# automerge/automerge-classic

Measured on NVIDIA H100. Metric: ops/sec applied (1M-op text trace), higher is better.
Workload: dtype int64

## Files before the change

### automerge_classic_b200/csrc/engine.cuh

```cuda
#pragma once
#include <algorithm>
#include <array>
#include <functional>
#include <initializer_list>
#include <map>
#include <memory>
#include <thread>
#include <zlib.h>
#include "patch.cuh"
#include "inflate.cuh"
#include "encode.cuh"
#include "prims.cuh"
#include "domlocal.cuh"
#include "doccols.cuh"
#include "history.cuh"
#include "unknowncols.hpp"

namespace amg {

struct DocBufs {
  DBuf<u64> id, obj, key; DBuf<u32> keyStrOff, keyStrLen, flags, valLen, valOff, time;
  void ensure(Ctx& c, size_t n, size_t keep = 0) {
    id.ensure(c, n, keep); obj.ensure(c, n, keep); key.ensure(c, n, keep); keyStrOff.ensure(c, n, keep); keyStrLen.ensure(c, n, keep);
    flags.ensure(c, n, keep); valLen.ensure(c, n, keep); valOff.ensure(c, n, keep); time.ensure(c, n, keep);
// ... 13 lines not shown
  size_t propsOff = 0, numProps = 0, editsOff = 0, numEdits = 0, elemOff = 0, valBytesOff = 0, valBytesLen = 0, bigEnd = 0;
  const u8* bytes = nullptr; size_t bytesLen = 0;
};

struct HostChange { u32 off, len; };

struct HostArena {
  HBuf<u8> buf; size_t len = 0;
  u8* data() { return buf.p; } const u8* data() const { return buf.p; }
  size_t size() const { return len; }
  void reserve(size_t n) { buf.ensure(n + 64); }
  void resize(size_t n) { if (n > len) buf.ensure(n + 64); len = n; }
  void append(const void* p, size_t n) { const size_t at = len; resize(len + n); memcpy(buf.p + at, p, n); }
  void assign(const HostArena& o) { resize(o.len); if (o.len) memcpy(buf.p, o.buf.p, o.len); }
};

inline std::string hex_of(const u8* p, size_t n) { static const char* d = "0123456789abcdef"; std::string s; for (size_t i = 0; i < n; i++) { s.push_back(d[p[i] >> 4]); s.push_back(d[p[i] & 15]); } return s; }

class Engine {
 public:
  Ctx ctx;
  DBuf<u8> arena; size_t arenaLen = 0; HostArena hostArena;
  DBuf<u8> hashes; size_t numApplied = 0;
  DocBufs doc; size_t numRows = 0; DBuf<u32> succOff; DBuf<u64> succ; size_t numSucc = 0;
  DBuf<ActorSlot> actorSlots; size_t actorCap = 0;
  DBuf<u32> actorRank;
  std::vector<std::string> actorIds;
  std::vector<u64> clock;
  std::vector<std::array<u8, 32>> heads; std::vector<u32> headIdx;
  std::vector<std::pair<u32, u32>> actorRep;
  std::vector<HostChange> changes;
  std::vector<std::array<u8, 32>> changeHashes;
  struct OrigRange { u32 idx; HostChange range; };
  std::vector<OrigRange> deflatedOriginal;
  const HostChange* originalOf(u32 idx) const {
    auto it = std::lower_bound(deflatedOriginal.begin(), deflatedOriginal.end(), idx, [](const OrigRange& a, u32 v) { return a.idx < v; });
    return it != deflatedOriginal.end() && it->idx == idx ? &it->range : nullptr;
  }
  std::vector<HostChange> queue, queueOriginal;
  u64 maxOp = 0;
  float lastPhaseMs[24] = {0};
  struct PhaseTimer* curTimer = nullptr; std::function<void()> curHostMark;
  std::vector<std::pair<const char*, float>> dbgMarks; std::function<void(const char*)> dbgMark = [](const char*) {};
  HBuf<u8> patchBuf;
  DBuf<u32> chOff, chLen, nOps, nPreds, nDeps, nActors, colOff, colLen, depBase, depIdx, primary, pass, flagWord, appRank, opBase, predBase, timeBase, amapBase, amap, authorSlot, newSlots;
  DBuf<u8> applied; DBuf<ChangeHot> hot; DBuf<ChangeMeta> meta ; DBuf<u64> errWord; DBuf<u32> hashTable;
  DBuf<u32> inflCap, inflCapOff, inflOvf; DBuf<u8> inflScratch;
  DBuf<u32> rawBase, rawPredBase, decErr, decDirect; DBuf<u64> decCursor; size_t lastDeflCount = 0, lastDeflStart = 0;
  u32* decTotalsPtr() { return reinterpret_cast<u32*>(decCursor.p + 2); }
  DBuf<u32> patchByteLen, patchByteOff; DBuf<u8> patchBytesD;
  DBuf<u32> r_objActor, r_objCtr, r_keyActor, r_keyCtr, r_keyStrOff, r_keyStrLen, r_insert, r_action, r_valLen, r_valOff, r_predNum, r_predOff, r_predActor, r_predCtr;
  DBuf<u64> o_id, o_obj, o_key, o_predId; DBuf<u32> o_keyStrOff, o_keyStrLen, o_flags, o_valLen, o_valOff, o_predOff, o_predNum, o_change, o_time;
  DBuf<u32> isRow, rowSlot, rowOfOp; DocBufs work, sorted;
  DBuf<u64> idKeys; DBuf<u32> idVals; DBuf<u32> objRow, elemRow, parentRow, keySlot, repList, repCount, listPos, perm, pos;
  DBuf<KeySlot> keySlots; DBuf<u64> sortKeys; DBuf<u32> sortVals; SortTemp sortTmp; ScanTemp scanTmp;
  ParColumnDecoder parCols{ctx, scanTmp}; size_t parDocMinRows = 4096;
  DBuf<u32> eNext, eRank, insItems, itemIdx, objSlot; DBuf<u64> ePacked, ePacked2;
  DBuf<u64> pairKey, pairSucc, newSucc; DBuf<u32> pairIdx, pairPos, pairTime, succCnt, newSuccCnt, newSuccOff, firstNewSucc;
  DBuf<u32> elemPos, keyRankAt, objPos, head, headScan, groupOf, groupRows, groupVisible, groupFirst, groupTouched, groupLinked, objTouchedAt, linkDone, emit, marker, slot;
  DBuf<u32> isObjHead, objIdx, objStart, elemVis, elemVisScan, rowEmit, firstVis, state, nItems, itemBase, qIndex, zero, wzero, zscan, wscan, editObjKey;
  DBuf<DomItem> items, items2; DBuf<PropRec> propOut; DBuf<EditRec> editOut, editOut2; DBuf<u64> editElem, editElem2;
  std::unique_ptr<ColumnEncoder> encoder; DBuf<long long> saveVals; DBuf<u32> saveStrOff, saveStrLen; std::string loadedDoc; size_t numLoaded = 0; HostChange loadedCols[9] = {}; DBuf<u64> counterTotal; DBuf<int> domW, domW2; DBuf<u32> elemMinT, editRowPos, editRowPos2, editObjKey2, rowClass, firstBare, counterOwner, newSuccTime, counterLast, runHeadFlag, runScan, runStart, elemFollower, domTw, domTw2, oldVisScan, inflLen, inflOff, groupHasChild, gCount, gElem, gT1, gQOrd, gBase, nQ, elemHasRecs, listLinkTime, editElemPos, editElemPos2, editKind, editPred, editDead, editMerge, editMulti, editLive;
  DBuf<u32> seqSlot, actorCnt, actorBaseD, clockD, changeActor, editTime; DBuf<u8> hashTmp; DBuf<u32> headsPack, headsOut; bool batchInOrder = true;
  DBuf<u32> finalTime, gFailed, memberFinal, opAt, runHead, opGroupHead; DBuf<u64> gBound; DocRows workView{}; DBuf<HostChange> chPairs; DBuf<u32> largeFlag, largeSlot, largeList; size_t lastNumLarge = 0; DBuf<u64> zwScan; DBuf<u32> deflList, patchTriples;

  explicit Engine(int device) {
    ctx.device = device;
#ifndef AMG_EMU
    int count = 0; cudaError_t e = cudaGetDeviceCount(&count);
    if (e != cudaSuccess || count == 0) throw Error(AMG_ERR_CUDA, "amgpu: no CUDA device available (this library has no CPU fallback)");
    CUDA_CHECK(cudaSetDevice(device));
    cudaDeviceProp prop; CUDA_CHECK(cudaGetDeviceProperties(&prop, device)); ctx.numSMs = prop.multiProcessorCount;
    CUDA_CHECK(cudaStreamCreateWithFlags(&ctx.stream, cudaStreamNonBlocking));
    CUDA_CHECK(cudaStreamCreateWithFlags(&ctx.side, cudaStreamNonBlocking));
    CUDA_CHECK(cudaStreamCreateWithFlags(&ctx.copy, cudaStreamNonBlocking));
    ctx.peekCap = 1u << 20; CUDA_CHECK(cudaMallocHost((void**)&ctx.peekBuf, ctx.peekCap + 64));
    ctx.peekFlag = reinterpret_cast<volatile unsigned long long*>(ctx.peekBuf + ctx.peekCap); *ctx.peekFlag = 0;
    CUDA_CHECK(cudaEventCreateWithFlags(&ctx.evUp, cudaEventDisableTiming)); CUDA_CHECK(cudaEventCreateWithFlags(&ctx.evMirror, cudaEventDisableTiming));
    CUDA_CHECK(cudaEventCreateWithFlags(&ctx.evFork, cudaEventDisableTiming)); CUDA_CHECK(cudaEventCreateWithFlags(&ctx.evJoin, cudaEventDisableTiming));
    ShaConsts k; memcpy(k.k, SHA_K, sizeof(SHA_K)); CUDA_CHECK(cudaMemcpyToSymbol(c_sha, &k, sizeof(k)));
#endif
    errWord.ensure(ctx, 4); flagWord.ensure(ctx, 16);
    actorCap = 64; actorSlots.ensure(ctx, actorCap); resetActorSlots(0, actorCap);
    succOff.ensure(ctx, 1); dev_memset(ctx, succOff.p, 0, 4);
  }
  ~Engine() {
#ifndef AMG_EMU
    if (ctx.stream) cudaStreamDestroy(ctx.stream);
    mirror_wait(ctx);
    if (ctx.side) cudaStreamDestroy(ctx.side);
    if (ctx.copy) cudaStreamDestroy(ctx.copy);
    if (ctx.peekBuf) cudaFreeHost(ctx.peekBuf);
    if (ctx.phaseEvReady) for (auto& e : ctx.phaseEv) cudaEventDestroy(e);
    if (last_peek_ctx() == &ctx) last_peek_ctx() = nullptr;
    if (ctx.evUp) cudaEventDestroy(ctx.evUp);
    if (ctx.evMirror) cudaEventDestroy(ctx.evMirror);
    if (ctx.evFork) cudaEventDestroy(ctx.evFork);
    if (ctx.evJoin) cudaEventDestroy(ctx.evJoin);
#endif
  }

  void rebuildActorTable() {
    std::vector<ActorSlot> t(actorCap); for (auto& s : t) { s.hash = 0; s.first = ~0ULL; s.actorNum = EMPTY32; s.repOff = 0; s.repLen = 0; s.pad = 0; }
    for (size_t a = 0; a < actorIds.size(); a++) {
      const u64 h = fnv1a64((const u8*)actorIds[a].data(), (u32)actorIds[a].size()); u64 s = mix64(h) & (actorCap - 1);
      while (t[s].hash != 0) s = (s + 1) & (actorCap - 1);
      t[s].hash = h; t[s].first = 0; t[s].actorNum = (u32)a; t[s].repOff = actorRep[a].first; t[s].repLen = actorRep[a].second;
    }
    h2d(ctx, actorSlots.p, t.data(), actorCap * sizeof(ActorSlot)); sync(ctx);
  }
// ... 138 lines not shown
```

### automerge_classic_b200/csrc/engine_impl.cuh

```cuda
#pragma once
#include <chrono>
#ifndef AMG_EMU
#include <nvtx3/nvToolsExt.h>
#endif
#include "engine.cuh"
#include "misc.cuh"

namespace amg {

#ifdef AMG_EMU
#define CUDA_CHECK_EMU(x) do {} while (0)
#else
#define CUDA_CHECK_EMU(x) CUDA_CHECK(x)
#endif
static const size_t PATCH_HDR_WORDS = 20;
struct NvtxPhases {
#ifndef AMG_EMU
  bool open = false;
  void next(const char* name) { if (open) nvtxRangePop(); open = name != nullptr; if (name) nvtxRangePushA(name); }
  ~NvtxPhases() { if (open) nvtxRangePop(); }
#else
  void next(const char*) {}
#endif
};
// ... 466 lines not shown
    if (!inOrder) {
      perm.ensure(ctx, B + 1); dev_memset(ctx, perm.p, 0, (B + 1) * 4);
      foreach(ctx, B, OpsInOrderKernel{nOps.p, applied.p, appRank.p, perm.p});
      scan_exclusive(ctx, scanTmp, perm.p, perm.p, numNew);
    }
    foreach(ctx, B, TimeBaseKernel{perm.p, applied.p, appRank.p, opBaseP, inOrder ? 1 : 0, timeBase.p});
    DBuf<u64>& maxOpD = pairSucc; maxOpD.ensure(ctx, 1); h2d(ctx, maxOpD.p, &maxOpNow, 8);
    foreach(ctx, B, MaxOpKernel{hot.p, nOps.p, applied.p, decErr.p, maxOpD.p, errWord.p});
    d2h(ctx, &maxOpNow, maxOpD.p, 8);
    RawRows raw = rawRows();
    lastNumLarge = 0;
    if (anyLarge) {
      largeFlag.ensure(ctx, B + 1); largeSlot.ensure(ctx, B + 2); largeList.ensure(ctx, B + 1);
      foreach(ctx, B, LargeFlagKernel{nOps.p, applied.p, largeFlag.p});
      scan_exclusive(ctx, scanTmp, largeFlag.p, largeSlot.p, B);
      lastNumLarge = readU32(largeSlot.p + B);
      if (lastNumLarge > 0) {
        foreach(ctx, B, CompactKernel{largeFlag.p, largeSlot.p, largeList.p});
        u32 hugeMask = 0;
        if (lastNumLarge <= 8) hugeMask = decodeHugeChanges(raw, lastNumLarge);
        foreach(ctx, (size_t)NCOLS * lastNumLarge, DecodeColumnKernel{arena.p, largeList.p, lastNumLarge, hot.p, nOps.p, nPreds.p, rawBase.p, rawPredBase.p, applied.p, raw, errWord.p, hugeDone.p});
        (void)hugeMask;
      }
    }
    for (DBuf<u64>* b : {&o_id, &o_obj, &o_key}) b->ensure(ctx, M + 1);
    o_predId.ensure(ctx, P + 1);
    for (DBuf<u32>* b : {&o_keyStrOff, &o_keyStrLen, &o_flags, &o_valLen, &o_valOff, &o_predOff, &o_predNum, &o_change, &o_time}) b->ensure(ctx, M + 1);
    OpRows ops{o_id.p, o_obj.p, o_key.p, o_keyStrOff.p, o_keyStrLen.p, o_flags.p, o_valLen.p, o_valOff.p, o_predOff.p, o_predNum.p, o_change.p, o_time.p, o_predId.p};
    foreach(ctx, M, FinalizeOpsKernel{B, hot.p, nActors.p, opBaseP, predBaseP, rawBase.p, rawPredBase.p, timeBase.p, amapBase.p, amap.p, applied.p, raw, ops, errWord.p});
    checkErr(actorsNow);
    dbgMark("decode:finalized");
    timer.mark(); hostMark(); nvtx.next("opset");
    if (maxOpNow >= (1ULL << 40)) throw Error(AMG_ERR_UNSUPPORTED, "amgpu: op counters above 2^40");
    const int ordBits = bits_for(maxOpNow) + rb;
    isRow.ensure(ctx, M + 1); rowSlot.ensure(ctx, M + 1); rowOfOp.ensure(ctx, M + 1);
    foreach(ctx, M, RowFlagKernel{o_flags.p, isRow.p}); scan_exclusive(ctx, scanTmp, isRow.p, rowSlot.p, M);
    const size_t R = readU32(rowSlot.p + M); N = numRows + R;
    if (N >= (1u << 29)) throw Error(AMG_ERR_UNSUPPORTED, "amgpu: more than 2^29 document rows");
    doc.ensure(ctx, N + 1, numRows);
    DocRows w = doc.view();
    foreach(ctx, M, AppendRowsKernel{ops, isRow.p, rowSlot.p, numRows, w, rowOfOp.p});
    const size_t icap = pow2_at_least(2 * N + 2); idKeys.ensure(ctx, icap); idVals.ensure(ctx, icap); dev_memset(ctx, idKeys.p, 0, icap * 8);
    idt = IdTable{idKeys.p, idVals.p, (u64)icap - 1};
    foreach(ctx, N, IdInsertKernel{w.id, idt, errWord.p});
    objRow.ensure(ctx, N + 1); elemRow.ensure(ctx, N + 1); parentRow.ensure(ctx, N + 1);
    foreach(ctx, N, ResolveRowsKernel{w, idt, ord, numRows, objRow.p, elemRow.p, parentRow.p, errWord.p});
    checkErr(actorsNow);
    dbgMark("opset:resolved");
    const size_t kcap = pow2_at_least(2 * N + 2); keySlots.ensure(ctx, kcap); keySlot.ensure(ctx, N + 1); repList.ensure(ctx, N + 1); repCount.ensure(ctx, 4);
    foreach(ctx, kcap, KeySlotInitKernel{keySlots.p});
    foreach(ctx, N, KeyInternKernel{arena.p, w, keySlots.p, (u64)kcap - 1, keySlot.p});
    dev_memset(ctx, repCount.p, 0, 16);
    foreach(ctx, N, KeyVerifyKernel{arena.p, w, keySlots.p, keySlot.p, repList.p, repCount.p, errWord.p});
    u32 rc[2]; readU32x2(repCount.p, repCount.p + 1, &rc[0], &rc[1]);
    const size_t D = rc[0]; const u32 maxKeyLen = rc[1];
    dbgMark("opset:keys-interned");
    if (D > 0) {
      sortKeys.ensure(ctx, D); sortVals.ensure(ctx, D);
      d2d(ctx, sortVals.p, repList.p, D * 4);
      const int chunks = (int)((maxKeyLen + 6) / 7);
      for (int ch = std::max(chunks, 1) - 1; ch >= 0; ch--) {
        foreach(ctx, D, KeyChunkKernel{arena.p, w, sortVals.p, (u32)ch * 7, sortKeys.p});
        sortPairs(sortKeys, sortVals, D, 64);
      }
      foreach(ctx, D, KeyRankKernel{sortVals.p, keySlot.p, keySlots.p});
    }
    listPos.ensure(ctx, N + 1); insItems.ensure(ctx, N + 1); emit.ensure(ctx, N + 1); slot.ensure(ctx, N + 2);
    foreach(ctx, N, InsertFlagKernel{w, emit.p}); scan_exclusive(ctx, scanTmp, emit.p, slot.p, N);
    const size_t I = readU32(slot.p + N);
    dbgMark("opset:inserts-counted");
    if (I > 0) {
      const int parentBits = bits_for(N) + 1;
      if (ordBits + parentBits > 64) throw Error(AMG_ERR_UNSUPPORTED, "amgpu: opId range x document size exceeds the 64-bit sibling sort key");
      foreach(ctx, N, CompactKernel{emit.p, slot.p, insItems.p});
      sortKeys.ensure(ctx, I); sortVals.ensure(ctx, I);
      foreach(ctx, I, SiblingKeyKernel{w, insItems.p, parentRow.p, objRow.p, ord, ordBits, sortKeys.p, errWord.p});
      d2d(ctx, sortVals.p, insItems.p, I * 4);
      sortPairs(sortKeys, sortVals, I, ordBits + parentBits);
      checkErr(actorsNow);
      itemIdx.ensure(ctx, N + 1); objSlot.ensure(ctx, N + 2);
      foreach(ctx, I, ItemIndexKernel{sortVals.p, itemIdx.p});
      foreach(ctx, N, ListObjFlagKernel{w, emit.p}); scan_exclusive(ctx, scanTmp, emit.p, objSlot.p, N);
      const size_t Lo = readU32(objSlot.p + N);
      const size_t S = 2 * I + 2 * Lo; eNext.ensure(ctx, S + 1); eRank.ensure(ctx, S + 1); ePacked.ensure(ctx, S + 1); ePacked2.ensure(ctx, S + 1);
      foreach(ctx, S, EulerInitKernel{eNext.p, eRank.p});
      foreach(ctx, I, EulerLinkKernel{sortKeys.p, ordBits, itemIdx.p, objSlot.p, eNext.p, eRank.p, I});
      foreach(ctx, S, ListRankPackKernel{eNext.p, eRank.p, ePacked.p});
      const int rounds = bits_for(S);
      for (int k = 0; k < rounds; k++) {
        foreach(ctx, S, ListRankPackedKernel{ePacked.p, ePacked2.p});
        std::swap(ePacked.p, ePacked2.p); std::swap(ePacked.cap, ePacked2.cap);
      }
      foreach(ctx, S, ListRankUnpackKernel{ePacked.p, eRank.p});
      foreach(ctx, N, ListPosKernel{eRank.p, elemRow.p, objRow.p, itemIdx.p, objSlot.p, (u32)I, listPos.p});
    } else dev_memset(ctx, listPos.p, 0, (N + 1) * 4);
    checkErr(actorsNow);
    dbgMark("opset:list-ranked");
    perm.ensure(ctx, N + 1); pos.ensure(ctx, N + 1); sortKeys.ensure(ctx, N);
    foreach(ctx, N, IotaKernel{perm.p});
    const int fieldBits[3] = {ordBits + 1, bits_for(N), ordBits + 1};
    for (int f = 0; f < 3; f++) {
      foreach(ctx, N, DocKeyKernel{f, w, perm.p, listPos.p, keySlots.p, keySlot.p, ord, sortKeys.p});
      sortPairs(sortKeys, perm, N, fieldBits[f]);
    }
    foreach(ctx, N, InversePermKernel{perm.p, pos.p});
    dbgMark("opset:doc-ordered(enqueued)");
    numPairs = numSucc + P;
    pairKey.ensure(ctx, numPairs + 1); pairSucc.ensure(ctx, numPairs + 1); pairIdx.ensure(ctx, numPairs + 1); pairPos.ensure(ctx, numPairs + 1); pairTime.ensure(ctx, numPairs + 1);
    foreach(ctx, M, DelElemCheckKernel{ops, idt, w, errWord.p});
    checkErr(actorsNow);
    foreach(ctx, numRows, OldPairsKernel{succOff.p, succ.p, pos.p, ord, pairKey.p, pairIdx.p, pairSucc.p, pairPos.p, pairTime.p});
    foreach(ctx, M, PredPairsKernel{ops, idt, pos.p, rowOfOp.p, w, elemRow.p, keySlot.p, ord, pairKey.p, pairIdx.p, pairSucc.p, pairPos.p, pairTime.p, numSucc, errWord.p});
    foreach(ctx, M, DelKeyCheckKernel{arena.p, ops, idt, w, errWord.p});
    foreach(ctx, M, IncCheckKernel{ops, idt, w, arena.p, errWord.p});
    {
      const u64 w2 = fetchErr();
      if (w2) {
        if ((w2 & 0xff) == KE_PRED_MISSING) { u64 pid = 0; d2h(ctx, &pid, o_predId.p + (w2 >> 8), 8); sync(ctx); actorIds.swap(actorsNow); std::string t = opIdText(pid); actorIds.swap(actorsNow); throw Error(AMG_ERR_RANGE, "no matching operation for pred: " + t); }
        if ((w2 & 0xff) == KE_UNKNOWN_COUNTER) { u64 oid = 0; d2h(ctx, &oid, o_id.p + (w2 >> 8), 8); sync(ctx); actorIds.swap(actorsNow); std::string t = opIdText(oid); actorIds.swap(actorsNow); throw Error(AMG_ERR_RANGE, "increment operation " + t + " for unknown counter"); }
        throwKernelError(w2, actorsNow);
      }
    }
    sortPairs(pairKey, pairIdx, numPairs, ordBits);
    foreach(ctx, numPairs, PairPosKeyKernel{pairPos.p, pairIdx.p, pairKey.p});
    sortPairs(pairKey, pairIdx, numPairs, bits_for(N));
    succCnt.ensure(ctx, N + 2); newSuccCnt.ensure(ctx, N + 2); newSuccOff.ensure(ctx, N + 2); firstNewSucc.ensure(ctx, N + 2); newSucc.ensure(ctx, numPairs + 1);
    dev_memset(ctx, succCnt.p, 0, (N + 2) * 4); dev_memset(ctx, newSuccCnt.p, 0, (N + 2) * 4); dev_memset(ctx, firstNewSucc.p, 0xff, (N + 2) * 4);
    foreach(ctx, numPairs, CountSuccKernel{pairPos.p, succCnt.p});
    foreach(ctx, numPairs, NewSuccFlagKernel{pairPos.p, pairTime.p, newSuccCnt.p});
    foreach(ctx, numPairs, FirstSuccTimeKernel{pairPos.p, pairTime.p, firstNewSucc.p});
    scan_exclusive(ctx, scanTmp, succCnt.p, newSuccOff.p, N);
    newSuccTime.ensure(ctx, numPairs + 1);
    foreach(ctx, numPairs, WriteSuccKernel{pairIdx.p, pairSucc.p, newSucc.p, pairTime.p, newSuccTime.p});
    sorted.ensure(ctx, N + 1);
    foreach(ctx, N, GatherRowsKernel{w, sorted.view(), perm.p});
    dbgMark("opset:succ+gather(enqueued)");
    timer.mark(); hostMark(); nvtx.next("patch");
    if (wantPatch) {
      objPos.ensure(ctx, N + 1);
      foreach(ctx, N, ObjPosKernel{perm.p, objRow.p, pos.p, objPos.p});
      workView = w;
      buildPatch(sorted.view(), N, false, &ops, M, &idt, rowOfOp.p, pos.p, actorsNow, out, newSuccOff.p, newSucc.p);
    }
    checkErr(actorsNow);
    timer.mark(); hostMark(); nvtx.next("heads+commit");
    dbgMark("commit:begin");
    {
      DBuf<u32>& isDep = groupLinked; isDep.ensure(ctx, G + 1); dev_memset(ctx, isDep.p, 0, (G + 1) * 4);
      foreach(ctx, B, MarkDepsKernel{applied.p, nDeps.p, depBase.p, depIdx.p, isDep.p});
      emit.ensure(ctx, B + 1); slot.ensure(ctx, B + 2); objStart.ensure(ctx, B + 1);
      foreach(ctx, B, HeadFlag2Kernel{applied.p, isDep.p, numApplied, emit.p});
      scan_exclusive(ctx, scanTmp, emit.p, slot.p, B);
      foreach(ctx, B, CompactKernel{emit.p, slot.p, objStart.p});
      const u32 nOld = (u32)headIdx.size(); u32 cap = 64, nh = 0; std::vector<u32> pack;
      headsPack.ensure(ctx, nOld + 1);
      if (nOld) h2d(ctx, headsPack.p, headIdx.data(), nOld * 4);
      for (;;) {
        const size_t words = 1 + (size_t)nOld + 9 * (size_t)cap;
// ... 1071 lines not shown
```

### automerge_classic_b200/csrc/opset.cuh

```cuda
#pragma once
#include "gate.cuh"

namespace amg {

static const u32 ROW_NONE = 0xffffffffu;
static const u32 ACT_MAKE_MAP = 0, ACT_SET = 1, ACT_MAKE_LIST = 2, ACT_DEL = 3, ACT_MAKE_TEXT = 4, ACT_INC = 5, ACT_MAKE_TABLE = 6, ACT_LINK = 7;

struct DocRows {
  u64 *id, *obj, *key; u32 *keyStrOff, *keyStrLen, *flags, *valLen, *valOff, *time;
};

struct Ord {
  const u32* actorRank; int rb;
  HD u64 operator()(u64 id) const { return (id_ctr(id) << rb) | (u64)actorRank[id_actor(id)]; }
};

struct RowFlagKernel {
  const u32* flags; u32* isRow;
  HD void operator()(size_t i) const { isRow[i] = flags_action(flags[i]) != ACT_DEL ? 1u : 0u; }
};
struct AppendRowsKernel {
  OpRows ops; const u32* isRow; const u32* rowSlot ; size_t numOld; DocRows w; u32* rowOfOp;
  HD void operator()(size_t i) const {
    if (!isRow[i]) { rowOfOp[i] = ROW_NONE; return; }
// ... 46 lines not shown
      } else {
        er = id_lookup(t, key);
        if (er == ROW_NONE || w.obj[er] != obj || !(w.flags[er] & F_INSERT)) { if (r >= numOld) raise(errWord, KE_REF_ELEM, r); er = ROW_NONE; }
      }
    }
    elemRow[r] = er; parentRow[r] = pr;
  }
};

struct KeySlot { u64 hash; u32 rep; u32 rank; };
struct KeyInternKernel {
  const u8* arena; DocRows w; KeySlot* slots; u64 mask; u32* keySlot;
  HD void operator()(size_t r) const {
    if (w.keyStrLen[r] == NULL32) { keySlot[r] = ROW_NONE; return; }
    u64 h = fnv1a64(arena + w.keyStrOff[r], w.keyStrLen[r]) ^ ((u64)w.keyStrLen[r] << 48); if (h == 0) h = 1;
    u64 s = mix64(h) & mask;
    while (true) {
      const u64 cur = atomic_cas(&slots[s].hash, (u64)0, h);
      if (cur == 0 || cur == h) { atomic_min(&slots[s].rep, (u32)r); keySlot[r] = (u32)s; return; }
      s = (s + 1) & mask;
    }
  }
};
struct KeyVerifyKernel {
  const u8* arena; DocRows w; const KeySlot* slots; const u32* keySlot; u32* repList; u32* repCount ; u64* errWord;
  HD void operator()(size_t r) const {
    const u32 s = keySlot[r]; if (s == ROW_NONE) return;
    const u32 rep = slots[s].rep;
    if (rep == (u32)r) { repList[atomic_add(repCount, 1u)] = (u32)r; atomic_max(repCount + 1, w.keyStrLen[r]); return; }
    const u32 len = w.keyStrLen[r];
    bool same = len == w.keyStrLen[rep];
    for (u32 i = 0; same && i < len; i++) same = arena[w.keyStrOff[r] + i] == arena[w.keyStrOff[rep] + i];
    if (!same) raise(errWord, KE_HASH_COLLISION, r);
  }
};
HD u64 key_chunk(const u8* s, u32 len, u32 pos) {
  u64 v = 0; u32 n = 0;
  for (u32 i = 0; i < 7; i++) {
    u32 b = 0;
    if (pos + i < len) { b = s[pos + i]; n++; if (b == 0xEE || b == 0xEF) b += 5; else if (b >= 0xF0 && b <= 0xF4) b -= 2; }
    v = (v << 8) | b;
  }
  return (v << 8) | n;
}
struct KeyChunkKernel {
  const u8* arena; DocRows w; const u32* items ; u32 pos; u64* chunk;
  HD void operator()(size_t j) const { const u32 r = items[j]; chunk[j] = key_chunk(arena + w.keyStrOff[r], w.keyStrLen[r], pos); }
};
struct KeyRankKernel {
  const u32* items; const u32* keySlot; KeySlot* slots;
  HD void operator()(size_t j) const { slots[keySlot[items[j]]].rank = (u32)j; }
};

struct IotaKernel { u32* out; HD void operator()(size_t i) const { out[i] = (u32)i; } };
struct FillU32Kernel { u32* out; u32 v; HD void operator()(size_t i) const { out[i] = v; } };
struct FillU64Kernel { u64* out; u64 v; HD void operator()(size_t i) const { out[i] = v; } };
struct GatherU64Kernel { const u64* src; const u32* idx; u64* out; HD void operator()(size_t i) const { out[i] = src[idx[i]]; } };
struct InversePermKernel { const u32* perm; u32* inv; HD void operator()(size_t i) const { inv[perm[i]] = (u32)i; } };
struct HeadFlagKernel { const u64* a; const u64* b; u32* flag; HD void operator()(size_t j) const { flag[j] = (j == 0 || a[j] != a[j - 1] || (b && b[j] != b[j - 1])) ? 1u : 0u; } };

struct SiblingKeyKernel {
  DocRows w; const u32* items; const u32* parentRow; const u32* objRow; Ord ord; int ordBits; u64* key; u64* errWord;
  HD void operator()(size_t j) const {
    const u32 r = items[j]; const u32 pr = parentRow[r];
    if (pr == ROW_NONE && objRow[r] == ROW_NONE) { raise(errWord, KE_UNSUPPORTED_OP, r); key[j] = 0; return; }
    if (pr == ROW_NONE) { const u32 a = flags_action(w.flags[objRow[r]]); if (a != ACT_MAKE_LIST && a != ACT_MAKE_TEXT) { raise(errWord, KE_UNSUPPORTED_OP, r); key[j] = 0; return; } }
    const u64 parentCode = pr != ROW_NONE ? ((u64)pr << 1) : (((u64)objRow[r] << 1) | 1);
    const u64 maxOrd = (1ULL << ordBits) - 1;
    key[j] = (parentCode << ordBits) | (maxOrd - ord(w.id[r]));
  }
};
struct ListObjFlagKernel { DocRows w; u32* flag; HD void operator()(size_t r) const { const u32 a = flags_action(w.flags[r]); flag[r] = (a == ACT_MAKE_LIST || a == ACT_MAKE_TEXT) ? 1u : 0u; } };
struct ItemIndexKernel { const u32* items; u32* itemIdx; HD void operator()(size_t j) const { itemIdx[items[j]] = (u32)j; } };
struct EulerLinkKernel {
  const u64* key; int ordBits; const u32* itemIdx; const u32* objSlot; u32* next ; u32* weight; size_t n;
  HD void operator()(size_t j) const {
    const u64 pc = key[j] >> ordBits;
    const bool firstOfParent = j == 0 || (key[j - 1] >> ordBits) != pc, lastOfParent = j + 1 == n || (key[j + 1] >> ordBits) != pc;
    const u32 parentEnter = (pc & 1) ? (u32)(2 * n + 2 * objSlot[pc >> 1]) : 2 * itemIdx[pc >> 1], parentExit = parentEnter + 1;
    if (firstOfParent) next[parentEnter] = (u32)(2 * j);
    next[2 * j + 1] = lastOfParent ? parentExit : (u32)(2 * j + 2);
    weight[2 * j] = 1;
  }
};
struct EulerInitKernel {
  u32* next; u32* weight;
  HD void operator()(size_t s) const { next[s] = (s & 1) ? (u32)s : (u32)s + 1; weight[s] = 0; }
};
struct ListRankPackKernel { const u32* next; const u32* rank; u64* packed; HD void operator()(size_t s) const { packed[s] = (u64)next[s] | ((u64)rank[s] << 32); } };
struct ListRankPackedKernel {
  const u64* in; u64* out;
  HD void operator()(size_t s) const {
    const u64 me = in[s]; const u32 n = (u32)me;
    if (n == (u32)s) { out[s] = me; return; }
    const u64 nb = in[n];
    out[s] = (u64)(u32)nb | ((u64)((u32)(me >> 32) + (u32)(nb >> 32)) << 32);
  }
};
struct ListRankUnpackKernel { const u64* packed; u32* rank; HD void operator()(size_t s) const { rank[s] = (u32)(packed[s] >> 32); } };
struct ListPosKernel {
  const u32* rank; const u32* elemRow; const u32* objRow; const u32* itemIdx; const u32* objSlot; u32 numItems; u32* listPos;
  HD void operator()(size_t r) const {
    const u32 e = elemRow[r];
    if (e == ROW_NONE || objRow[e] == ROW_NONE) { listPos[r] = 0; return; }
    listPos[r] = rank[2 * (size_t)numItems + 2 * objSlot[objRow[e]]] - rank[2 * (size_t)itemIdx[e]];
  }
};

struct DocKeyKernel {
  int field; DocRows w; const u32* perm; const u32* listPos; const KeySlot* keySlots; const u32* keySlot; Ord ord; u64* key;
  HD void operator()(size_t j) const {
    const u32 r = perm[j]; u64 k;
    if (field == 0) k = (w.keyStrLen[r] == NULL32 && (w.flags[r] & F_INSERT)) ? 0 : ord(w.id[r]) + 1;
    else if (field == 1) k = w.keyStrLen[r] == NULL32 ? listPos[r] : keySlots[keySlot[r]].rank;
    else k = w.obj[r] == 0 ? 0 : ord(w.obj[r]) + 1;
    key[j] = k;
  }
};
struct GatherRowsKernel {
  DocRows src, dst; const u32* perm;
  HD void operator()(size_t p) const {
    const u32 r = perm[p];
    dst.id[p] = src.id[r]; dst.obj[p] = src.obj[r]; dst.key[p] = src.key[r]; dst.keyStrOff[p] = src.keyStrOff[r]; dst.keyStrLen[p] = src.keyStrLen[r];
    dst.flags[p] = src.flags[r]; dst.valLen[p] = src.valLen[r]; dst.valOff[p] = src.valOff[r]; dst.time[p] = src.time[r];
  }
};

struct PredPairsKernel {
  OpRows ops; IdTable t; const u32* pos ; const u32* rowOfOp; DocRows w; const u32* elemRow; const u32* keySlot;
  Ord ord; u64* pairKey ; u32* pairIdx; u64* pairSucc; u32* pairPos; u32* pairTime; size_t pairBase; u64* errWord;
  HD void operator()(size_t i) const {
    const u32 n = ops.predNum[i];
    for (u32 j = 0; j < n; j++) {
      const size_t p = ops.predOff[i] + j; const size_t q = pairBase + p;
      const u32 target = id_lookup(t, ops.predId[p]);
      pairKey[q] = ord(ops.id[i]); pairIdx[q] = (u32)q; pairSucc[q] = ops.id[i]; pairTime[q] = ops.time[i];
      if (target == ROW_NONE || (ops.flags[i] & F_INSERT)) { raise(errWord, KE_PRED_MISSING, p); pairPos[q] = 0; continue; }
      bool ok = w.obj[target] == ops.obj[i] && w.time[target] < ops.time[i] && ord(ops.predId[p]) < ord(ops.id[i]);
      if (ops.keyStrLen[i] != NULL32) {
        ok = ok && w.keyStrLen[target] != NULL32;
        const u32 r = rowOfOp[i];
        if (ok && r != ROW_NONE) ok = keySlot[r] == keySlot[target];
      } else {
        ok = ok && w.keyStrLen[target] == NULL32 && elemRow[target] != ROW_NONE && w.id[elemRow[target]] == ops.key[i];
      }
      if (!ok) raise(errWord, KE_PRED_MISSING, p);
      pairPos[q] = pos[target];
    }
  }
};
struct IncCheckKernel {
  OpRows ops; IdTable t; DocRows w; const u8* arena; u64* errWord;
  HD void operator()(size_t i) const {
    const u32 act = flags_action(ops.flags[i]), tag = ops.valLen[i] & 15;
    if ((act == ACT_INC || (act == ACT_SET && tag == 8)) && (tag == 3 || tag == 4 || tag == 8 || tag == 9)) {
      ByteReader r(arena, ops.valOff[i], ops.valOff[i] + (ops.valLen[i] >> 4));
      if (tag == 3) r.uleb(); else r.sleb();
      if (r.err) raise(errWord, r.err, i);
    }
    if (act != ACT_INC) return;
    if (tag > 4 && tag != 8 && tag != 9) { raise(errWord, KE_UNSUPPORTED_OP, i); return; }
    bool ok = false, other = false;
    for (u32 j = 0; j < ops.predNum[i]; j++) {
      const u32 target = id_lookup(t, ops.predId[ops.predOff[i] + j]);
      if (target != ROW_NONE && flags_action(w.flags[target]) == ACT_SET && (w.valLen[target] & 15) == 8) ok = true; else other = true;
    }
    if (!ok) raise(errWord, KE_UNKNOWN_COUNTER, i);
    else if (other) raise(errWord, KE_UNSUPPORTED_OP, i);
  }
// ... 42 lines not shown
```

Baseline: 151.7 million.

## Replace pointer-jumping list ranking and three-pass doc sort with splitter tour walk and placement

Result: faster. 162.0 million (median of 6 runs) (+6.8%).

```diff
diff --git a/automerge_classic_b200/csrc/engine.cuh b/automerge_classic_b200/csrc/engine.cuh
--- a/automerge_classic_b200/csrc/engine.cuh
+++ b/automerge_classic_b200/csrc/engine.cuh
@@ -89,10 +89,11 @@
   DBuf<u32> r_objActor, r_objCtr, r_keyActor, r_keyCtr, r_keyStrOff, r_keyStrLen, r_insert, r_action, r_valLen, r_valOff, r_predNum, r_predOff, r_predActor, r_predCtr;
   DBuf<u64> o_id, o_obj, o_key, o_predId; DBuf<u32> o_keyStrOff, o_keyStrLen, o_flags, o_valLen, o_valOff, o_predOff, o_predNum, o_change, o_time;
   DBuf<u32> isRow, rowSlot, rowOfOp; DocBufs work, sorted;
-  DBuf<u64> idKeys; DBuf<u32> idVals; DBuf<u32> objRow, elemRow, parentRow, keySlot, repList, repCount, listPos, perm, pos;
+  DBuf<u64> idKeys; DBuf<u32> idVals; DBuf<u32> objRow, elemRow, parentRow, keySlot, repList, repCount, perm, pos;
   DBuf<KeySlot> keySlots; DBuf<u64> sortKeys; DBuf<u32> sortVals; SortTemp sortTmp; ScanTemp scanTmp;
   ParColumnDecoder parCols{ctx, scanTmp}; size_t parDocMinRows = 4096;
-  DBuf<u32> eNext, eRank, insItems, itemIdx, objSlot; DBuf<u64> ePacked, ePacked2;
+  DBuf<u32> insItems, restItems, itemIdx, objSlot, childCnt, sibFlag, sibSlot, tourNext, tourW, tourRank; DBuf<u64> tourOwn;
+  DBuf<u32> objFlag, objFlagScan, objHead, objHeadScan, objRankOf, objElems, objRestStart, objCount, objBase;
   DBuf<u64> pairKey, pairSucc, newSucc; DBuf<u32> pairIdx, pairPos, pairTime, succCnt, newSuccCnt, newSuccOff, firstNewSucc;
   DBuf<u32> elemPos, keyRankAt, objPos, head, headScan, groupOf, groupRows, groupVisible, groupFirst, groupTouched, groupLinked, objTouchedAt, linkDone, emit, marker, slot;
   DBuf<u32> isObjHead, objIdx, objStart, elemVis, elemVisScan, rowEmit, firstVis, state, nItems, itemBase, qIndex, zero, wzero, zscan, wscan, editObjKey;
diff --git a/automerge_classic_b200/csrc/engine_impl.cuh b/automerge_classic_b200/csrc/engine_impl.cuh
--- a/automerge_classic_b200/csrc/engine_impl.cuh
+++ b/automerge_classic_b200/csrc/engine_impl.cuh
@@ -542,9 +542,21 @@
     foreach(ctx, N, KeyInternKernel{arena.p, w, keySlots.p, (u64)kcap - 1, keySlot.p});
     dev_memset(ctx, repCount.p, 0, 16);
     foreach(ctx, N, KeyVerifyKernel{arena.p, w, keySlots.p, keySlot.p, repList.p, repCount.p, errWord.p});
-    u32 rc[2]; readU32x2(repCount.p, repCount.p + 1, &rc[0], &rc[1]);
-    const size_t D = rc[0]; const u32 maxKeyLen = rc[1];
-    dbgMark("opset:keys-interned");
+    emit.ensure(ctx, N + 1); slot.ensure(ctx, N + 2); insItems.ensure(ctx, N + 1); restItems.ensure(ctx, N + 1); objSlot.ensure(ctx, N + 2);
+    foreach(ctx, N, InsertFlagKernel{w, emit.p}); scan_exclusive(ctx, scanTmp, emit.p, slot.p, N);
+    foreach(ctx, N, SplitRowsKernel{emit.p, slot.p, insItems.p, restItems.p});
+    const SiblingParent par{w, parentRow.p, objRow.p};
+    childCnt.ensure(ctx, 2 * N + 1); sibFlag.ensure(ctx, N + 1); sibSlot.ensure(ctx, N + 2);
+    dev_memset(ctx, childCnt.p, 0, 2 * N * 4);
+    foreach(ctx, N, SiblingCountKernel{par, emit.p, childCnt.p, errWord.p});
+    foreach(ctx, N, SiblingFlagKernel{par, emit.p, childCnt.p, sibFlag.p}); scan_exclusive(ctx, scanTmp, sibFlag.p, sibSlot.p, N);
+    foreach(ctx, N, ListObjFlagKernel{w, emit.p}); scan_exclusive(ctx, scanTmp, emit.p, objSlot.p, N);
+    objFlag.ensure(ctx, 2 * N + 1); objFlagScan.ensure(ctx, 2 * N + 2); objRankOf.ensure(ctx, 2 * N + 1);
+    dev_memset(ctx, objFlag.p, 0, 2 * N * 4);
+    foreach(ctx, N, ObjEntryFlagKernel{w, objRow.p, objFlag.p}); scan_exclusive(ctx, scanTmp, objFlag.p, objFlagScan.p, 2 * N);
+    u32 cnt[6]; { void* dst[6] = {&cnt[0], &cnt[1], &cnt[2], &cnt[3], &cnt[4], &cnt[5]}; readWords({{repCount.p, 4}, {repCount.p + 1, 4}, {slot.p + N, 4}, {objSlot.p + N, 4}, {objFlagScan.p + 2 * N, 4}, {sibSlot.p + N, 4}}, dst); }
+    const size_t D = cnt[0]; const u32 maxKeyLen = cnt[1]; const size_t I = cnt[2], Lo = cnt[3], numObjEntries = cnt[4], numSib = cnt[5], numRest = N - I;
+    dbgMark("opset:counted");
     if (D > 0) {
       sortKeys.ensure(ctx, D); sortVals.ensure(ctx, D);
       d2d(ctx, sortVals.p, repList.p, D * 4);
@@ -555,45 +567,73 @@
       }
       foreach(ctx, D, KeyRankKernel{sortVals.p, keySlot.p, keySlots.p});
     }
-    listPos.ensure(ctx, N + 1); insItems.ensure(ctx, N + 1); emit.ensure(ctx, N + 1); slot.ensure(ctx, N + 2);
-    foreach(ctx, N, InsertFlagKernel{w, emit.p}); scan_exclusive(ctx, scanTmp, emit.p, slot.p, N);
-    const size_t I = readU32(slot.p + N);
-    dbgMark("opset:inserts-counted");
+    if (numObjEntries > 0) {
+      sortKeys.ensure(ctx, numObjEntries); sortVals.ensure(ctx, numObjEntries); objHead.ensure(ctx, numObjEntries + 1); objHeadScan.ensure(ctx, numObjEntries + 1);
+      foreach(ctx, 2 * N, CompactKernel{objFlag.p, objFlagScan.p, sortVals.p});
+      foreach(ctx, numObjEntries, ObjEntryKeyKernel{w, sortVals.p, ord, sortKeys.p});
+      sortPairs(sortKeys, sortVals, numObjEntries, ordBits);
+      foreach(ctx, numObjEntries, HeadFlagKernel{sortKeys.p, nullptr, objHead.p}); scan_exclusive(ctx, scanTmp, objHead.p, objHeadScan.p, numObjEntries);
+      foreach(ctx, numObjEntries, ObjRankKernel{sortVals.p, objHead.p, objHeadScan.p, objRankOf.p});
+    }
     if (I > 0) {
       const int parentBits = bits_for(N) + 1;
       if (ordBits + parentBits > 64) throw Error(AMG_ERR_UNSUPPORTED, "amgpu: opId range x document size exceeds the 64-bit sibling sort key");
-      foreach(ctx, N, CompactKernel{emit.p, slot.p, insItems.p});
-      sortKeys.ensure(ctx, I); sortVals.ensure(ctx, I);
-      foreach(ctx, I, SiblingKeyKernel{w, insItems.p, parentRow.p, objRow.p, ord, ordBits, sortKeys.p, errWord.p});
-      d2d(ctx, sortVals.p, insItems.p, I * 4);
-      sortPairs(sortKeys, sortVals, I, ordBits + parentBits);
-      checkErr(actorsNow);
-      itemIdx.ensure(ctx, N + 1); objSlot.ensure(ctx, N + 2);
-      foreach(ctx, I, ItemIndexKernel{sortVals.p, itemIdx.p});
-      foreach(ctx, N, ListObjFlagKernel{w, emit.p}); scan_exclusive(ctx, scanTmp, emit.p, objSlot.p, N);
-      const size_t Lo = readU32(objSlot.p + N);
-      const size_t S = 2 * I + 2 * Lo; eNext.ensure(ctx, S + 1); eRank.ensure(ctx, S + 1); ePacked.ensure(ctx, S + 1); ePacked2.ensure(ctx, S + 1);
-      foreach(ctx, S, EulerInitKernel{eNext.p, eRank.p});
-      foreach(ctx, I, EulerLinkKernel{sortKeys.p, ordBits, itemIdx.p, objSlot.p, eNext.p, eRank.p, I});
-      foreach(ctx, S, ListRankPackKernel{eNext.p, eRank.p, ePacked.p});
-      const int rounds = bits_for(S);
-      for (int k = 0; k < rounds; k++) {
-        foreach(ctx, S, ListRankPackedKernel{ePacked.p, ePacked2.p});
-        std::swap(ePacked.p, ePacked2.p); std::swap(ePacked.cap, ePacked2.cap);
-      }
-      foreach(ctx, S, ListRankUnpackKernel{ePacked.p, eRank.p});
-      foreach(ctx, N, ListPosKernel{eRank.p, elemRow.p, objRow.p, itemIdx.p, objSlot.p, (u32)I, listPos.p});
-    } else dev_memset(ctx, listPos.p, 0, (N + 1) * 4);
+      if (numSib > 0) {
+        sortKeys.ensure(ctx, numSib); sortVals.ensure(ctx, numSib);
+        foreach(ctx, N, CompactKernel{sibFlag.p, sibSlot.p, sortVals.p});
+        foreach(ctx, numSib, SiblingKeyKernel{par, sortVals.p, ord, ordBits, sortKeys.p});
+        sortPairs(sortKeys, sortVals, numSib, ordBits + parentBits);
+      }
+    }
     checkErr(actorsNow);
+    const size_t numObjs = numObjEntries + 1;
+    objElems.ensure(ctx, numObjs + 1); dev_memset(ctx, objElems.p, 0, (numObjs + 1) * 4);
+    ListRank lr{nullptr, itemIdx.p, objSlot.p, objRow.p, (u32)I};
+    if (I > 0) {
+      itemIdx.ensure(ctx, N + 1); lr.itemIdx = itemIdx.p;
+      foreach(ctx, I, ItemIndexKernel{insItems.p, itemIdx.p});
+      const size_t S = 2 * I + 2 * Lo;
+      struct Level { u32 numIdx, numIdxSplit; size_t off, n; };
+      std::vector<Level> lv;
+      size_t top = 0;
+      for (u32 numIdx = (u32)(2 * I);;) {
+        const u32 numIdxSplit = numIdx <= TOUR_K ? 0 : 2 * ((numIdx + TOUR_K - 1) / TOUR_K);
+        const size_t n = lv.empty() ? S : numIdx + Lo;
+        lv.push_back({numIdx, numIdxSplit, top, n}); top += n;
+        if (!numIdxSplit) break;
+        numIdx = numIdxSplit;
+      }
+      tourNext.ensure(ctx, top + Lo + 1); tourW.ensure(ctx, top + Lo + 1); tourRank.ensure(ctx, top + 1); tourOwn.ensure(ctx, top + 1);
+      foreach(ctx, S, EulerInitKernel{tourNext.p});
+      foreach(ctx, I, EulerLinkKernel{par, insItems.p, childCnt.p, itemIdx.p, objSlot.p, tourNext.p, I});
+      foreach(ctx, numSib, EulerSiblingLinkKernel{sortKeys.p, sortVals.p, ordBits, itemIdx.p, objSlot.p, tourNext.p, I, numSib});
+      for (size_t L = 0; L < lv.size(); L++) {
+        const size_t up = L + 1 < lv.size() ? lv[L + 1].off : top;
+        foreach(ctx, lv[L].numIdxSplit + Lo, TourWalkKernel{tourNext.p + lv[L].off, L ? tourW.p + lv[L].off : nullptr, lv[L].numIdx, L ? 1u : 2u, lv[L].numIdxSplit,
+                                                          tourOwn.p + lv[L].off, tourNext.p + up, tourW.p + up});
+      }
+      for (size_t L = lv.size(); L-- > 0;)
+        foreach(ctx, lv[L].n, TourExpandKernel{tourOwn.p + lv[L].off, L + 1 < lv.size() ? tourRank.p + lv[L + 1].off : tourW.p + top, tourRank.p + lv[L].off});
+      lr.rank = tourRank.p;
+      foreach(ctx, N, ListElemsKernel{w, objFlag.p, objRankOf.p, lr, objElems.p});
+    }
     dbgMark("opset:list-ranked");
-    perm.ensure(ctx, N + 1); pos.ensure(ctx, N + 1); sortKeys.ensure(ctx, N);
-    foreach(ctx, N, IotaKernel{perm.p});
-    const int fieldBits[3] = {ordBits + 1, bits_for(N), ordBits + 1};
-    for (int f = 0; f < 3; f++) {
-      foreach(ctx, N, DocKeyKernel{f, w, perm.p, listPos.p, keySlots.p, keySlot.p, ord, sortKeys.p});
-      sortPairs(sortKeys, perm, N, fieldBits[f]);
-    }
-    foreach(ctx, N, InversePermKernel{perm.p, pos.p});
+    const int objBits = bits_for(numObjs), midBits = bits_for(std::max<size_t>(std::max(D, I), 1)), lowBits = ordBits + 1;
+    const bool twoSorts = objBits + midBits + lowBits > 64;
+    const int objShift = twoSorts ? midBits : midBits + lowBits, midShift = twoSorts ? 0 : lowBits;
+    sortKeys.ensure(ctx, numRest + 1); sortVals.ensure(ctx, numRest + 1);
+    d2d(ctx, sortVals.p, restItems.p, numRest * 4);
+    RestKeyKernel rk{w, sortVals.p, objRow.p, objRankOf.p, elemRow.p, lr, keySlots.p, keySlot.p, ord, midBits, twoSorts ? 0 : lowBits, twoSorts, sortKeys.p};
+    if (twoSorts) { foreach(ctx, numRest, rk); sortPairs(sortKeys, sortVals, numRest, lowBits); rk.lowOnly = false; }
+    rk.items = sortVals.p; rk.key = sortKeys.p;
+    foreach(ctx, numRest, rk);
+    sortPairs(sortKeys, sortVals, numRest, objShift + objBits);
+    objRestStart.ensure(ctx, numObjs + 1); objCount.ensure(ctx, numObjs + 1); objBase.ensure(ctx, numObjs + 2);
+    foreach(ctx, numObjs, ObjSpanKernel{sortKeys.p, (u32)numRest, objShift, objElems.p, objRestStart.p, objCount.p});
+    scan_exclusive(ctx, scanTmp, objCount.p, objBase.p, numObjs);
+    perm.ensure(ctx, N + 1); pos.ensure(ctx, N + 1);
+    foreach(ctx, numRest, PlaceRestKernel{sortKeys.p, sortVals.p, objShift, midShift, (u32)((1ull << midBits) - 1), objBase.p, objElems.p, objRestStart.p, perm.p, pos.p});
+    foreach(ctx, I, PlaceInsertKernel{insItems.p, objRow.p, objRankOf.p, lr, sortKeys.p, (u32)numRest, objShift, midShift, objBase.p, objRestStart.p, perm.p, pos.p});
     dbgMark("opset:doc-ordered(enqueued)");
     numPairs = numSucc + P;
     pairKey.ensure(ctx, numPairs + 1); pairSucc.ensure(ctx, numPairs + 1); pairIdx.ensure(ctx, numPairs + 1); pairPos.ensure(ctx, numPairs + 1); pairTime.ensure(ctx, numPairs + 1);
diff --git a/automerge_classic_b200/csrc/opset.cuh b/automerge_classic_b200/csrc/opset.cuh
--- a/automerge_classic_b200/csrc/opset.cuh
+++ b/automerge_classic_b200/csrc/opset.cuh
@@ -122,69 +122,150 @@
   HD void operator()(size_t j) const { slots[keySlot[items[j]]].rank = (u32)j; }
 };
 
-struct IotaKernel { u32* out; HD void operator()(size_t i) const { out[i] = (u32)i; } };
 struct FillU32Kernel { u32* out; u32 v; HD void operator()(size_t i) const { out[i] = v; } };
 struct FillU64Kernel { u64* out; u64 v; HD void operator()(size_t i) const { out[i] = v; } };
 struct GatherU64Kernel { const u64* src; const u32* idx; u64* out; HD void operator()(size_t i) const { out[i] = src[idx[i]]; } };
-struct InversePermKernel { const u32* perm; u32* inv; HD void operator()(size_t i) const { inv[perm[i]] = (u32)i; } };
 struct HeadFlagKernel { const u64* a; const u64* b; u32* flag; HD void operator()(size_t j) const { flag[j] = (j == 0 || a[j] != a[j - 1] || (b && b[j] != b[j - 1])) ? 1u : 0u; } };
-
+HD u32 lower_bound_u64(const u64* k, u32 n, u64 v) { u32 lo = 0, hi = n; while (lo < hi) { const u32 m = (lo + hi) >> 1; if (k[m] < v) lo = m + 1; else hi = m; } return lo; }
+
+struct SiblingParent {
+  DocRows w; const u32* parentRow; const u32* objRow;
+  HD u64 operator()(u32 r) const {
+    const u32 pr = parentRow[r];
+    if (pr != ROW_NONE) return (u64)pr << 1;
+    if (objRow[r] == ROW_NONE) return ~0ULL;
+    const u32 a = flags_action(w.flags[objRow[r]]);
+    return (a == ACT_MAKE_LIST || a == ACT_MAKE_TEXT) ? (((u64)objRow[r] << 1) | 1) : ~0ULL;
+  }
+};
+struct SiblingCountKernel {
+  SiblingParent par; const u32* isInsert; u32* childCnt; u64* errWord;
+  HD void operator()(size_t r) const {
+    if (!isInsert[r]) return;
+    const u64 pc = par((u32)r);
+    if (pc == ~0ULL) { raise(errWord, KE_UNSUPPORTED_OP, r); return; }
+    atomic_add(&childCnt[pc], 1u);
+  }
+};
+struct SiblingFlagKernel {
+  SiblingParent par; const u32* isInsert; const u32* childCnt; u32* flag;
+  HD void operator()(size_t r) const { u32 f = 0; if (isInsert[r]) { const u64 pc = par((u32)r); f = pc != ~0ULL && childCnt[pc] > 1 ? 1u : 0u; } flag[r] = f; }
+};
 struct SiblingKeyKernel {
-  DocRows w; const u32* items; const u32* parentRow; const u32* objRow; Ord ord; int ordBits; u64* key; u64* errWord;
-  HD void operator()(size_t j) const {
-    const u32 r = items[j]; const u32 pr = parentRow[r];
-    if (pr == ROW_NONE && objRow[r] == ROW_NONE) { raise(errWord, KE_UNSUPPORTED_OP, r); key[j] = 0; return; }
-    if (pr == ROW_NONE) { const u32 a = flags_action(w.flags[objRow[r]]); if (a != ACT_MAKE_LIST && a != ACT_MAKE_TEXT) { raise(errWord, KE_UNSUPPORTED_OP, r); key[j] = 0; return; } }
-    const u64 parentCode = pr != ROW_NONE ? ((u64)pr << 1) : (((u64)objRow[r] << 1) | 1);
-    const u64 maxOrd = (1ULL << ordBits) - 1;
-    key[j] = (parentCode << ordBits) | (maxOrd - ord(w.id[r]));
-  }
+  SiblingParent par; const u32* items; Ord ord; int ordBits; u64* key;
+  HD void operator()(size_t j) const { const u32 r = items[j]; key[j] = (par(r) << ordBits) | (((1ULL << ordBits) - 1) - ord(par.w.id[r])); }
 };
 struct ListObjFlagKernel { DocRows w; u32* flag; HD void operator()(size_t r) const { const u32 a = flags_action(w.flags[r]); flag[r] = (a == ACT_MAKE_LIST || a == ACT_MAKE_TEXT) ? 1u : 0u; } };
 struct ItemIndexKernel { const u32* items; u32* itemIdx; HD void operator()(size_t j) const { itemIdx[items[j]] = (u32)j; } };
+HD u32 euler_enter(u64 pc, size_t numItems, const u32* itemIdx, const u32* objSlot) { return (pc & 1) ? (u32)(2 * numItems + 2 * objSlot[pc >> 1]) : 2 * itemIdx[pc >> 1]; }
 struct EulerLinkKernel {
-  const u64* key; int ordBits; const u32* itemIdx; const u32* objSlot; u32* next ; u32* weight; size_t n;
+  SiblingParent par; const u32* items; const u32* childCnt; const u32* itemIdx; const u32* objSlot; u32* next ; size_t n;
   HD void operator()(size_t j) const {
-    const u64 pc = key[j] >> ordBits;
-    const bool firstOfParent = j == 0 || (key[j - 1] >> ordBits) != pc, lastOfParent = j + 1 == n || (key[j + 1] >> ordBits) != pc;
-    const u32 parentEnter = (pc & 1) ? (u32)(2 * n + 2 * objSlot[pc >> 1]) : 2 * itemIdx[pc >> 1], parentExit = parentEnter + 1;
-    if (firstOfParent) next[parentEnter] = (u32)(2 * j);
-    next[2 * j + 1] = lastOfParent ? parentExit : (u32)(2 * j + 2);
-    weight[2 * j] = 1;
+    const u64 pc = par(items[j]);
+    if (childCnt[pc] != 1) return;
+    const u32 parentEnter = euler_enter(pc, n, itemIdx, objSlot);
+    next[parentEnter] = (u32)(2 * j); next[2 * j + 1] = parentEnter + 1;
+  }
+};
+struct EulerSiblingLinkKernel {
+  const u64* key; const u32* sorted; int ordBits; const u32* itemIdx; const u32* objSlot; u32* next; size_t numItems, n;
+  HD void operator()(size_t m) const {
+    const u64 pc = key[m] >> ordBits;
+    const bool firstOfParent = m == 0 || (key[m - 1] >> ordBits) != pc, lastOfParent = m + 1 == n || (key[m + 1] >> ordBits) != pc;
+    const u32 parentEnter = euler_enter(pc, numItems, itemIdx, objSlot), me = 2 * itemIdx[sorted[m]];
+    if (firstOfParent) next[parentEnter] = me;
+    next[me + 1] = lastOfParent ? parentEnter + 1 : 2 * itemIdx[sorted[m + 1]];
   }
 };
 struct EulerInitKernel {
-  u32* next; u32* weight;
-  HD void operator()(size_t s) const { next[s] = (s & 1) ? (u32)s : (u32)s + 1; weight[s] = 0; }
-};
-struct ListRankPackKernel { const u32* next; const u32* rank; u64* packed; HD void operator()(size_t s) const { packed[s] = (u64)next[s] | ((u64)rank[s] << 32); } };
-struct ListRankPackedKernel {
-  const u64* in; u64* out;
-  HD void operator()(size_t s) const {
-    const u64 me = in[s]; const u32 n = (u32)me;
-    if (n == (u32)s) { out[s] = me; return; }
-    const u64 nb = in[n];
-    out[s] = (u64)(u32)nb | ((u64)((u32)(me >> 32) + (u32)(nb >> 32)) << 32);
-  }
-};
-struct ListRankUnpackKernel { const u64* packed; u32* rank; HD void operator()(size_t s) const { rank[s] = (u32)(packed[s] >> 32); } };
-struct ListPosKernel {
-  const u32* rank; const u32* elemRow; const u32* objRow; const u32* itemIdx; const u32* objSlot; u32 numItems; u32* listPos;
-  HD void operator()(size_t r) const {
-    const u32 e = elemRow[r];
-    if (e == ROW_NONE || objRow[e] == ROW_NONE) { listPos[r] = 0; return; }
-    listPos[r] = rank[2 * (size_t)numItems + 2 * objSlot[objRow[e]]] - rank[2 * (size_t)itemIdx[e]];
-  }
-};
-
-struct DocKeyKernel {
-  int field; DocRows w; const u32* perm; const u32* listPos; const KeySlot* keySlots; const u32* keySlot; Ord ord; u64* key;
+  u32* next;
+  HD void operator()(size_t s) const { next[s] = (s & 1) ? (u32)s : (u32)s + 1; }
+};
+
+static const u32 TOUR_K = 16;
+struct TourWalkKernel {
+  const u32* next; const u32* weight ;
+  u32 numIdx, headStride, numIdxSplit ;
+  u64* own ; u32* upNext; u32* upWeight;
+  HD bool isSplitter(u32 s) const { return s < numIdx ? (numIdxSplit != 0 && s % TOUR_K < 2) : (s - numIdx) % headStride == 0; }
+  HD u32 splitterId(u32 s) const { return s < numIdx ? 2 * (s / TOUR_K) + s % TOUR_K : numIdxSplit + (s - numIdx) / headStride; }
+  HD void operator()(size_t t) const {
+    u32 s = t < numIdxSplit ? (u32)(t >> 1) * TOUR_K + (u32)(t & 1) : numIdx + ((u32)t - numIdxSplit) * headStride, acc = 0;
+    while (true) {
+      own[s] = ((u64)t << 32) | acc;
+      acc += weight ? weight[s] : (s < numIdx && !(s & 1)) ? 1u : 0u;
+      const u32 n = next[s];
+      if (n == s) { upNext[t] = (u32)t; break; }
+      if (isSplitter(n)) { upNext[t] = splitterId(n); break; }
+      s = n;
+    }
+    upWeight[t] = acc;
+  }
+};
+struct TourExpandKernel { const u64* own; const u32* upRank; u32* rank; HD void operator()(size_t s) const { const u64 o = own[s]; rank[s] = upRank[o >> 32] - (u32)o; } };
+struct ListRank {
+  const u32* rank; const u32* itemIdx; const u32* objSlot; const u32* objRow; u32 numItems;
+  HD u32 total(u32 listObj) const { return rank[2 * (size_t)numItems + 2 * objSlot[listObj]]; }
+  HD u32 before(u32 e) const { return total(objRow[e]) - rank[2 * (size_t)itemIdx[e]]; }
+};
+
+struct ObjEntryFlagKernel {
+  DocRows w; const u32* objRow; u32* flag ;
+  HD void operator()(size_t r) const {
+    if (w.obj[r] == 0) return;
+    const u32 o = objRow[r]; u32* f = flag + (o != ROW_NONE ? 2 * (size_t)o : 2 * r + 1);
+    if (!*f) *f = 1u;
+  }
+};
+struct ObjEntryKeyKernel { DocRows w; const u32* entries; Ord ord; u64* key; HD void operator()(size_t j) const { const u32 e = entries[j], r = e >> 1; key[j] = ord((e & 1) ? w.obj[r] : w.id[r]); } };
+struct ObjRankKernel { const u32* entries; const u32* head; const u32* headScan; u32* rankOf; HD void operator()(size_t j) const { rankOf[entries[j]] = headScan[j] + head[j]; } };
+HD u32 obj_rank(const DocRows& w, const u32* objRow, const u32* rankOf, size_t r) {
+  if (w.obj[r] == 0) return 0;
+  const u32 o = objRow[r]; return rankOf[o != ROW_NONE ? 2 * (size_t)o : 2 * r + 1];
+}
+struct SplitRowsKernel {
+  const u32* isInsert; const u32* insSlot; u32* insItems; u32* restItems;
+  HD void operator()(size_t r) const { if (isInsert[r]) insItems[insSlot[r]] = (u32)r; else restItems[r - insSlot[r]] = (u32)r; }
+};
+struct RestKeyKernel {
+  DocRows w; const u32* items; const u32* objRow; const u32* rankOf; const u32* elemRow; ListRank lr ;
+  const KeySlot* keySlots; const u32* keySlot; Ord ord; int midBits, lowBits; bool lowOnly; u64* key;
   HD void operator()(size_t j) const {
-    const u32 r = perm[j]; u64 k;
-    if (field == 0) k = (w.keyStrLen[r] == NULL32 && (w.flags[r] & F_INSERT)) ? 0 : ord(w.id[r]) + 1;
-    else if (field == 1) k = w.keyStrLen[r] == NULL32 ? listPos[r] : keySlots[keySlot[r]].rank;
-    else k = w.obj[r] == 0 ? 0 : ord(w.obj[r]) + 1;
-    key[j] = k;
+    const u32 r = items[j]; const u64 low = ord(w.id[r]) + 1;
+    if (lowOnly) { key[j] = low; return; }
+    u32 mid;
+    if (w.keyStrLen[r] != NULL32) mid = keySlots[keySlot[r]].rank;
+    else { const u32 e = elemRow[r]; mid = (e == ROW_NONE || objRow[e] == ROW_NONE || !lr.rank) ? 0 : lr.before(e); }
+    const u64 high = ((u64)obj_rank(w, objRow, rankOf, r) << midBits) | mid;
+    key[j] = lowBits ? (high << lowBits) | low : high;
+  }
+};
+struct ListElemsKernel {
+  DocRows w; const u32* objFlag; const u32* rankOf; ListRank lr; u32* nElem;
+  HD void operator()(size_t r) const { const u32 a = flags_action(w.flags[r]); if ((a == ACT_MAKE_LIST || a == ACT_MAKE_TEXT) && objFlag[2 * r]) nElem[rankOf[2 * r]] = lr.total((u32)r); }
+};
+struct ObjSpanKernel {
+  const u64* restKey; u32 numRest; int objShift; const u32* nElem; u32* restStart; u32* count;
+  HD void operator()(size_t o) const {
+    const u32 a = lower_bound_u64(restKey, numRest, (u64)o << objShift), b = lower_bound_u64(restKey, numRest, (u64)(o + 1) << objShift);
+    restStart[o] = a; count[o] = nElem[o] + (b - a);
+  }
+};
+struct PlaceRestKernel {
+  const u64* key; const u32* items; int objShift, midShift; u32 midMask; const u32* objBase; const u32* nElem; const u32* restStart; u32* perm; u32* pos;
+  HD void operator()(size_t j) const {
+    const u64 k = key[j]; const u32 o = (u32)(k >> objShift), mid = (u32)(k >> midShift) & midMask;
+    const u32 p = objBase[o] + (mid < nElem[o] ? mid + 1 : nElem[o]) + ((u32)j - restStart[o]), r = items[j];
+    perm[p] = r; pos[r] = p;
+  }
+};
+struct PlaceInsertKernel {
+  const u32* items; const u32* objRow; const u32* rankOf; ListRank lr; const u64* restKey; u32 numRest; int objShift, midShift;
+  const u32* objBase; const u32* restStart; u32* perm; u32* pos;
+  HD void operator()(size_t j) const {
+    const u32 r = items[j], o = rankOf[2 * (size_t)objRow[r]], f = lr.before(r);
+    const u32 p = objBase[o] + f + (lower_bound_u64(restKey, numRest, ((u64)o << objShift) | ((u64)f << midShift)) - restStart[o]);
+    perm[p] = r; pos[r] = p;
   }
 };
 struct GatherRowsKernel {
```
